# nirajbabar/raytracinginonesemester

Measured on AMD Instinct MI355X. Metric: Mrays/s at 1920x1080x16spp (1/2/4/8 GPU) + PPM max-abs pixel diff, higher is better.
Workload: dtype f32+f64

## Files before the change

raytracinginonesemester_amd/csrc/rt_device.hip:

```cpp

#include <hip/hip_runtime.h>
#include <hip/hip_ext.h>

#include <cfloat>
#include <cmath>
#include <cstdint>
#include <cstdio>
#include <cstdlib>
#include <cstring>
#include <algorithm>
#include <atomic>
#include <functional>
#include <memory>
#include <new>
#include <string>
#include <array>
#include <vector>

#include "rt_common.hpp"
#include "rt_hip_host.hpp"
#include "rt_math.hpp"
#include "rt_ppm.hpp"
#include "rt_scene_pack.hpp"
#include "rt_tilediv.hpp"
// ... 52 lines not shown
    int32_t lane_wide;
    const float* __restrict__ cut;
    int32_t ncut;
    const float* __restrict__ cut2;
    int32_t cut_sub_log2;
    const float4* __restrict__ tri;
    uint32_t* fault;
};

__device__ __forceinline__ f3 scene_bmax(const SceneView& sc) { return mk(sc.bmax[0], sc.bmax[1], sc.bmax[2]); }

struct RenderParams {
    SceneView sc;
    f3 cam_center, cam_p00, cam_du, cam_dv;
    int32_t W, H, spp, max_depth, diffuse_bounce;
    f3 miss;
    const float* __restrict__ jitter;
    int32_t band_rows, band_index, band_count, rows;
    int32_t tile_w, tile_h, tiles_x, tiles_total;
    int32_t lane_samples;
    int32_t half_waves;
    int32_t paired_only;
    int32_t tile_order;
    int32_t spp_log2, tile_w_log2;
    int32_t cull;
    f3 miss_pixel;
    uint32_t* live_count;
    int32_t* live_tiles;
    int32_t* cut_tiles;
    uint32_t* next_count;
    int32_t cut_force;
    int32_t nqueues;
    int32_t queue_cap;
    uint32_t tiles_x_mul;
    float* __restrict__ rgb;
    int32_t* __restrict__ hit_idx;
    float* __restrict__ hit_t;
    uint8_t* __restrict__ p6;
    uint8_t miss_p6[4];
    uint32_t tiles_x_shift;
    uint16_t* __restrict__ tile_cost;
    int32_t* heavy_tiles;
    int32_t heavy_cap;
    uint32_t heavy_ticks[8];
    unsigned long long* ray_count;
    uint32_t* drained;
    uint32_t drain_tag;
    int32_t gate_q8;
};
static_assert(sizeof(RenderParams) == 544, "RenderParams: a field moved");

#include "rt_wave.hpp"
#include "rt_instrument.hpp"
#include "rt_traverse.hpp"
#include "rt_shade.hpp"
#include "rt_prepass.hpp"
#include "rt_query.hpp"
#include "rt_multihit.hpp"
#include "rt_closest.hpp"
#include "rt_path.hpp"
#include "rt_refit.hpp"
#include "rt_rebuild.hpp"

__device__ __forceinline__ int work_length(const RenderParams& P, int q, int& heavy) {
    heavy = 0;
    if (P.heavy_cap > 0)
        for (int k = 0; k < NCLASS; ++k) heavy += min((int)ldc_u32(P.live_count + heavy_counter(k, q)), P.heavy_cap);
    const int slot = P.sc.ncut > 0 ? CUT_SLOT0 + q : q;
    return heavy + (int)ldc_u32(&P.live_count[slot * COUNTER_STRIDE]);
}

__device__ __forceinline__ int work_tile(const RenderParams& P, int q, int e, int heavy, int& cls) {
    const uint32_t* list;
    cls = NCLASS;
    if (e < heavy) {
        int k = 0;
        for (; k < NCLASS - 1; ++k) {
            const int n = min((int)ldc_u32(P.live_count + heavy_counter(k, q)), P.heavy_cap);
            if (e < n) break;
            e -= n;
        }
        list = reinterpret_cast<const uint32_t*>(P.heavy_tiles) + ((size_t)k * 8 + q) * P.heavy_cap;
        cls = k;
    } else {
        e -= heavy;
        list = reinterpret_cast<const uint32_t*>(P.sc.ncut > 0 ? P.cut_tiles : P.live_tiles) + (size_t)q * P.queue_cap;
    }
    return (int)ldc_u32(list + e);
}

__device__ __forceinline__ uint32_t dequeue(uint32_t* head, uint32_t lane) {
    uint32_t v = 0;
    if (lane == 0) v = __hip_atomic_fetch_add(head, 1u, __ATOMIC_RELAXED, __HIP_MEMORY_SCOPE_AGENT);
    return uni(v);
}

template <int MODE, bool D1, int LS = 0>
__device__ __forceinline__ void samples_tile(const RenderParams& P, int tile, uint32_t qw, int t, float* col,
                                             int* kpix, float* park, const int* lds_zero) {
    const uint32_t wv = uni((uint32_t)t) >> 6;
    constexpr int wl = LS != 0 ? 32 : 64;
    const bool on = (t & 63) < wl;
    const int lt = ((int)qw * wl) | (t & (wl - 1));
    bool all_miss = false;
    {
        const int s = lt & (P.spp - 1);
        const int pit = lt >> P.spp_log2;
        int tx, ty;
        if constexpr (D1) {
            ty = (int)tile_div((uint32_t)tile, TileDiv{P.tiles_x_mul, P.tiles_x_shift});
            tx = tile - ty * P.tiles_x;
        } else {
            tx = tile % P.tiles_x;
            ty = tile / P.tiles_x;
        }
#ifndef RT_ROW_PIXELS
        int px, py;
        if (P.tile_w == P.tile_h) {
            px = (pit & 1) | ((pit >> 1) & 2) | ((pit >> 2) & 4) | ((pit >> 3) & 8);
            py = ((pit >> 1) & 1) | ((pit >> 2) & 2) | ((pit >> 3) & 4) | ((pit >> 4) & 8);
        } else {
            px = pit & (P.tile_w - 1);
            py = pit >> P.tile_w_log2;
        }
#else
        const int px = pit & (P.tile_w - 1), py = pit >> P.tile_w_log2;
#endif
        const int x = tx * P.tile_w + px;
        const int r = ty * P.tile_h + py;
        const bool valid = on && x < P.W && r < P.rows;
        const int y = valid ? global_row(P, r) : 0;
        const int pix = valid ? r * P.W + x : -1;
        if (s == 0) kpix[t >> P.spp_log2] = pix;
        const int64_t aov = valid && P.hit_idx ? (int64_t)pix * P.spp + s : -1;
        if constexpr (D1) RT_PHASE_ITEM(park + (wv << 6), (uint32_t)tile * (BLOCK / 64) + qw);
        const f3 c = trace_sample<MODE, D1, LS == 3 ? 2 : 0>(P, valid, x, y, s, aov, park + t,
                                                                             park + (wv << 6));
        if constexpr (D1) RT_PHASE(park + (wv << 6), 1);
        if constexpr (D1) all_miss = P.spp <= 64 && !d1_wave_hit(park + (wv << 6));
        if (!all_miss) {
            const int te = (int)((wv << 6) | __builtin_amdgcn_mbcnt_hi(~0u, __builtin_amdgcn_mbcnt_lo(
                                                      ~0u, (uint32_t)*(const volatile int*)lds_zero)));
            col[3 * te] = c.x;
            col[3 * te + 1] = c.y;
            col[3 * te + 2] = c.z;
        }
    }
    const int t2 = (int)((wv << 6) | __builtin_amdgcn_mbcnt_hi(~0u, __builtin_amdgcn_mbcnt_lo(
                                             ~0u, (uint32_t)*(const volatile int*)lds_zero)));
    if (P.spp <= 64) {
        __builtin_amdgcn_fence(__ATOMIC_RELEASE, "wavefront");
        __builtin_amdgcn_wave_barrier();
        __builtin_amdgcn_fence(__ATOMIC_ACQUIRE, "wavefront");
    } else {
        __syncthreads();
    }
    if (D1 && P.spp <= 64) {
        const int ppw_log2 = 6 - P.spp_log2;
        const float rs = __int_as_float((127 - P.spp_log2) << 23);
        for (int i = t2 & 63; i < (3 << ppw_log2); i += 64) {
            const int ch = i >> ppw_log2, pw = i & ((1 << ppw_log2) - 1);
            const int pix = kpix[(int)(wv << ppw_log2) + pw];
            if (pix < 0) continue;
            const size_t k = (size_t)pix * 3 + ch;
            if (all_miss) {
                const uint32_t m0 = uni((uint32_t)__float_as_int(P.miss_pixel.x)),
                               m1 = uni((uint32_t)__float_as_int(P.miss_pixel.y)),
                               m2 = uni((uint32_t)__float_as_int(P.miss_pixel.z));
                uint32_t b;
                __builtin_memcpy(&b, P.miss_p6, sizeof(b));
                b = uni(b);
                if (P.rgb) P.rgb[k] = __int_as_float((int)(ch == 0 ? m0 : ch == 1 ? m1 : m2));
                if (P.p6) P.p6[k] = (uint8_t)(b >> (8 * ch));
                continue;
            }
            const float* sp = col + 3 * (int)((wv << 6) + ((uint32_t)pw << P.spp_log2)) + ch;
            float acc = 0.f;
            int j = 0;
            for (; j + 16 <= P.spp; j += 16) {
                float s[16];
#pragma unroll
                for (int u = 0; u < 16; ++u) s[u] = sp[3 * (j + u)];
#pragma unroll
                for (int u = 0; u < 16; ++u) acc = acc + s[u];
            }
            for (; j + 4 <= P.spp; j += 4) {
                float s[4];
#pragma unroll
                for (int u = 0; u < 4; ++u) s[u] = sp[3 * (j + u)];
#pragma unroll
                for (int u = 0; u < 4; ++u) acc = acc + s[u];
            }
            for (; j < P.spp; ++j) acc = acc + sp[3 * j];
            const float v = acc * rs;
            if (P.rgb) P.rgb[k] = v;
            if (P.p6) P.p6[k] = rtp::p6_default_sample(v);
        }
        if constexpr (D1) RT_PHASE(park + (wv << 6), 3);
        return;
    }
    if ((t2 & (P.spp - 1)) == 0) {
        const int pix = kpix[t2 >> P.spp_log2];
        if (pix >= 0) {
            f3 acc = mk(0.f, 0.f, 0.f);
            for (int k = 0; k < P.spp; ++k)
                acc = add(acc, mk(col[3 * (t2 + k)], col[3 * (t2 + k) + 1], col[3 * (t2 + k) + 2]));
            const float rs = 1.0f / (float)P.spp;
            const size_t k = (size_t)pix * 3;
            const f3 px = mk(acc.x * rs, acc.y * rs, acc.z * rs);
            if (P.rgb) {
                P.rgb[k] = px.x;
                P.rgb[k + 1] = px.y;
                P.rgb[k + 2] = px.z;
            }
            if (P.p6) {
                P.p6[k] = rtp::p6_default_sample(px.x);
                P.p6[k + 1] = rtp::p6_default_sample(px.y);
                P.p6[k + 2] = rtp::p6_default_sample(px.z);
            }
        }
    }
    if constexpr (D1) RT_PHASE(park + (wv << 6), 3);
}

template <int MODE, bool D1>
__device__ __forceinline__ void pixels_tile(const RenderParams& P, int tile, uint32_t qw, int tid, float* park) {
    const int t = (int)((qw << 6) | (tid & 63));
    const int tx = tile % P.tiles_x, ty = tile / P.tiles_x;
    const int x = tx * P.tile_w + t % P.tile_w;
    const int r = ty * P.tile_h + t / P.tile_w;
    const bool valid = x < P.W && r < P.rows;
    const int y = valid ? global_row(P, r) : 0;
    f3 acc = mk(0.f, 0.f, 0.f);
    if constexpr (D1) RT_PHASE_ITEM(park + (uni((uint32_t)tid) & ~63u), (uint32_t)tile * (BLOCK / 64) + qw);
    for (int s = 0; s < P.spp; ++s) {
        const int64_t aov = valid && P.hit_idx ? ((int64_t)r * P.W + x) * P.spp + s : -1;
        acc = add(acc, trace_sample<MODE, D1>(P, valid, x, y, s, aov, park + tid, park + (uni((uint32_t)tid) & ~63u)));
    }
    if (valid) {
        const float fs = (float)P.spp;
        const size_t k = ((size_t)r * P.W + x) * 3;
        const f3 px = mk(acc.x / fs, acc.y / fs, acc.z / fs);
        if (P.rgb) {
            P.rgb[k] = px.x;
            P.rgb[k + 1] = px.y;
            P.rgb[k + 2] = px.z;
        }
        if (P.p6) {
            P.p6[k] = rtp::p6_default_sample(px.x);
            P.p6[k + 1] = rtp::p6_default_sample(px.y);
            P.p6[k + 2] = rtp::p6_default_sample(px.z);
        }
    }
}

#ifndef RT_RENDER_WAVES
#define RT_RENDER_WAVES 7
#endif
#ifndef RT_BOUNCE_WAVES
#define RT_BOUNCE_WAVES 3
#endif
#ifndef RT_PAIRED_WAVES
#define RT_PAIRED_WAVES 4
#endif
#ifndef RT_RENDER_WAVES_BIG
#define RT_RENDER_WAVES_BIG 8
#endif
struct PairParams {
    RenderParams f[2];
};

__global__ __launch_bounds__(BLOCK) void tile_cull_pair_kernel(PairParams PP) {
    __builtin_amdgcn_s_setprio(3);
    const int nba = (PP.f[0].tiles_total + BLOCK - 1) / BLOCK;
    const bool b = (int)blockIdx.x >= nba;
    const RenderParams& P = b ? PP.f[1] : PP.f[0];
    const int bx = b ? (int)blockIdx.x - nba : (int)blockIdx.x;
    if (bx == 0 && threadIdx.x < COUNTER_SLOTS) P.next_count[threadIdx.x * COUNTER_STRIDE] = 0u;
    cull_tiles(P, bx * BLOCK + (int)threadIdx.x);
}

__global__ __launch_bounds__(BLOCK) void tile_cut_pair_kernel(PairParams PP) {
    __shared__ CutScratch scratch[BLOCK / 64];
    __builtin_amdgcn_s_setprio(3);
    const uint32_t lane = lane_id();
    const int wib = (int)uni(threadIdx.x / 64);
    const int wave = (int)(blockIdx.x * (BLOCK / 64)) + wib;
    const int waves = (int)(gridDim.x * (BLOCK / 64)) / 2;
    const RenderParams& P = (wave & 1) ? PP.f[1] : PP.f[0];
    float box[6] = {0.f, 0.f, 0.f, -1.f, -1.f, -1.f};
    int max_len;
    const bool test = cut_setup(P, lane, box, max_len);
    for (int p = wave >> 1;; p += waves) {
        const int q = p % P.nqueues, g = p / P.nqueues;
        if (CUT_GROUP * g >= max_len) break;
        (void)cut_unit(P, lane, q, g, test, box, scratch[wib]);
    }
}

__device__ __forceinline__ int pair_tile(const RenderParams& A, const RenderParams& B, int q, int e, int& which,
                                         int& cls) {
    for (int k = 0; k < NCLASS; ++k) {
        const int na = A.heavy_cap > 0 ? min((int)ldc_u32(A.live_count + heavy_counter(k, q)), A.heavy_cap) : 0;
        if (e < na) {
            which = 0;
            cls = k;
            return (int)ldc_u32(reinterpret_cast<const uint32_t*>(A.heavy_tiles) + ((size_t)k * 8 + q) * A.heavy_cap + e);
        }
        e -= na;
        const int nb = B.heavy_cap > 0 ? min((int)ldc_u32(B.live_count + heavy_counter(k, q)), B.heavy_cap) : 0;
        if (e < nb) {
            which = 1;
            cls = k;
            return (int)ldc_u32(reinterpret_cast<const uint32_t*>(B.heavy_tiles) + ((size_t)k * 8 + q) * B.heavy_cap + e);
        }
        e -= nb;
    }
    cls = NCLASS;
    const int ra = (int)ldc_u32(&A.live_count[(A.sc.ncut > 0 ? CUT_SLOT0 + q : q) * COUNTER_STRIDE]);
    which = e < ra ? 0 : 1;
    const RenderParams& X = e < ra ? A : B;
    if (e >= ra) e -= ra;
    return (int)ldc_u32(reinterpret_cast<const uint32_t*>(X.sc.ncut > 0 ? X.cut_tiles : X.live_tiles) +
                        (size_t)q * X.queue_cap + e);
}

template <int MODE, bool SAMPLES, bool D1, int WAVES, int LS, bool PAIR>
__device__ __forceinline__ void render_tiles_body() {
    constexpr int WPT = BLOCK / 64;
    __shared__ float col[SAMPLES ? BLOCK * 3 : 1];
    __shared__ int kpix[SAMPLES ? BLOCK : 1];
    __shared__ float park[D1 ? PARK_SLOTS * BLOCK
                             : (MODE == RT_KERNEL_LANE || (MODE & MODE_DEEP) != 0 ? 1 : LANE_LDS_CAP * BLOCK)];
    __shared__ uint32_t t_start[WPT], t_item[WPT];
    __shared__ int lds_zero;
    __shared__ uint32_t block_item;
    if constexpr (SAMPLES) lds_zero = 0;
    const uint32_t wv = uni((uint32_t)threadIdx.x) >> 6;
    for (bool first = true;; first = false) {
        typedef const __attribute__((address_space(4))) RenderParams* KernargP;
        KernargP pp = (KernargP)__builtin_amdgcn_kernarg_segment_ptr();
        uint32_t bx = blockIdx.x;
        asm volatile("" : "+s"(pp), "+s"(bx));
        const RenderParams& R0 = *(const RenderParams*)pp;
        const RenderParams& RG = PAIR ? *(const RenderParams*)(pp + 1) : R0;
        const int g = (int)(bx & 7);
        const int q = R0.nqueues == 1 ? 0 : g;
        uint32_t* head = R0.live_count + (HEAD_SLOT0 + g) * COUNTER_STRIDE;
        const bool blockwise = SAMPLES && R0.spp > 64;
        const uint32_t lane = fresh_lane_id();
        RT_HOOK_FRAME_FIRST(first, lane, RG);
        const int tid = (int)((wv << 6) | lane);
        const uint32_t per_queue = (gridDim.x >> 3) * (blockwise ? 1u : (uint32_t)WPT);
        uint32_t j;
        if (first) {
            j = (bx >> 3) * (blockwise ? 1u : (uint32_t)WPT) + (blockwise ? 0u : wv);
        } else if (blockwise) {
            if (tid == 0) block_item = dequeue(head, lane);
            __syncthreads();
            j = per_queue + uni(block_item);
        } else {
            j = per_queue + dequeue(head, lane);
        }
        int heavy;
        int n = work_length(R0, q, heavy);
        if constexpr (PAIR) {
            int hb;
            n += work_length(RG, q, hb);
        }
        const int e = (R0.nqueues == 1 ? g : 0) + (R0.nqueues == 1 ? 8 : 1) * (int)(blockwise ? j : j / WPT);
        if (RG.drained && lane == 0) {
            const int ge = (int)(((int64_t)n * RG.gate_q8) >> 8);
            if (e >= ge && e < ge + (R0.nqueues == 1 ? 8 : 1))
                __hip_atomic_store(RG.drained, RG.drain_tag, __ATOMIC_RELAXED, __HIP_MEMORY_SCOPE_SYSTEM);
        }
        if (e >= n) {
            RT_HOOK_FRAME_LAST(lane, RG);
            break;
        }
        const uint32_t qw = blockwise ? wv : j % WPT;
        int cls;
        KernargP pr = pp;
        int tile;
        if constexpr (PAIR) {
            int which;
            tile = pair_tile(R0, RG, q, e, which, cls);
            pr = pp + which;
        } else {
            tile = work_tile(R0, q, e, heavy, cls);
        }
        const RenderParams& R = *(const RenderParams*)pr;
        if (cls == 0) __builtin_amdgcn_s_setprio(3);
        else if (cls == 1) __builtin_amdgcn_s_setprio(2);
        else if (cls == 2) __builtin_amdgcn_s_setprio(1);
        else __builtin_amdgcn_s_setprio(0);
        RT_HOOK_ITEM_START(wt0);
        if (R.tile_cost && lane == 0) {
            t_start[wv] = (uint32_t)wall_clock64();
            t_item[wv] = (uint32_t)tile * WPT + qw;
        }
        if constexpr (SAMPLES) samples_tile<MODE, D1, LS>(R, tile, qw, tid, col, kpix, park, &lds_zero);
        else pixels_tile<MODE, D1>(R, tile, qw, tid, park);
        if (R.tile_cost && fresh_lane_id() == 0) {
            asm volatile("" ::: "memory");
            const uint32_t d = (uint32_t)wall_clock64() - t_start[wv];
            R.tile_cost[t_item[wv]] = (uint16_t)(d < 0xffffu ? d : 0xffffu);
        }
        RT_HOOK_ITEM_END(wt0, tile, WPT, qw, bx, first, wv);
    }
}

template <int MODE, bool SAMPLES, bool D1, int WAVES = RT_RENDER_WAVES, int LS = 0>
__global__ __launch_bounds__(BLOCK, WAVES) void render_tiles_kernel(RenderParams P) {
    render_tiles_body<MODE, SAMPLES, D1, WAVES, LS, false>();
}

template <int MODE, bool SAMPLES, bool D1, int WAVES = RT_RENDER_WAVES, int LS = 0>
__global__ __launch_bounds__(BLOCK, WAVES) void render_pair_kernel(PairParams P) {
    render_tiles_body<MODE, SAMPLES, D1, WAVES, LS, true>();
}

__global__ __launch_bounds__(BLOCK) void powf_kernel(const float* __restrict__ x, const float* __restrict__ y, int n,
                                                     float* __restrict__ out) {
    const int i = (int)(blockIdx.x * BLOCK + threadIdx.x);
    if (i < n) out[i] = ref_powf(x[i], y[i]);
}

__global__ __launch_bounds__(BLOCK) void box_test_kernel(const float* __restrict__ rays, const float* __restrict__ boxes,
                                                         const float* __restrict__ tminmax,
                                                         const float* __restrict__ bmax,
                                                         const uint8_t* __restrict__ active, int n,
                                                         int32_t* __restrict__ out) {
    const int i = (int)(blockIdx.x * BLOCK + threadIdx.x);
    const bool in = i < n;
    const size_t j = (size_t)(in ? i : n - 1);
    const float* R = rays + 6 * j;
    const float* B = boxes + 6 * j;
    f3 bm;
    if (bmax != nullptr) {
        bm = mk(bmax[3 * j], bmax[3 * j + 1], bmax[3 * j + 2]);
    } else {
        bm = mk(fmaxf(fabsf(B[0]), fabsf(B[3])), fmaxf(fabsf(B[1]), fabsf(B[4])), fmaxf(fabsf(B[2]), fabsf(B[5])));
        if (!(B[0] <= B[3] && B[1] <= B[4] && B[2] <= B[5])) bm = mk(INFINITY, INFINITY, INFINITY);
    }
    const BoxP b = {(v2f){B[0], B[3]}, (v2f){B[1], B[4]}, (v2f){B[2], B[5]}};
    const float tmin = tminmax[2 * j], tmax = tminmax[2 * j + 1];
    const RayPre r = make_ray(mk(R[0], R[1], R[2]), mk(R[3], R[4], R[5]), bm, tmin);
    const RayPre rw = make_ray(r.o, r.d, bm);
    const uint64_t act = ballot(in && (active == nullptr || active[j] != 0));
    const int cls = box_classify(r, b, tmax);
    const bool h = box_hit(r, b, tmin, tmax);
    const uint64_t m0 = box_hit_mask<false, false>(rw, b, tmax, act);
    const uint64_t m1 = box_hit_mask<true, false>(rw, b, tmax, act);
    const uint64_t m2 = box_hit_mask<true, true>(rw, b, tmax, act);
    if (in) {
        int32_t* O = out + 5 * j;
        O[0] = h ? 1 : 0;
        O[1] = cls;
        O[2] = lane_in(m0) ? 1 : 0;
        O[3] = lane_in(m1) ? 1 : 0;
        O[4] = lane_in(m2) ? 1 : 0;
// ... 1578 lines not shown
    const int slot = int((s->launches - 1) % rt_scene::kRing);
    HIP_TRY(hipEventSynchronize(s->ev1[slot]));
    uint32_t c[COUNTER_SET_U32];
    const size_t counter_bytes = COUNTER_SET_U32 * sizeof(uint32_t);
    HIP_TRY(hipMemcpy(c, static_cast<const char*>(s->work.p) + ((s->launches - 1) % rt_scene::kSets) * counter_bytes, sizeof(c),
                      hipMemcpyDeviceToHost));
    for (int k = 0; k < 8; ++k) *live += c[k * COUNTER_STRIDE];
    if (heavy) {
        *heavy = 0;
        if (s->last_heavy_cap > 0)
            for (int k = 0; k < 8 * NCLASS; ++k)
                *heavy += std::min<int64_t>(c[(HEAVY_SLOT0 + k) * COUNTER_STRIDE], s->last_heavy_cap);
    }
    return RT_OK;
}
}

extern "C" int rt_live_tiles(const rt_scene* s, int64_t* live, int64_t* total) {
    return live_tiles(s, live, nullptr, total);
}

extern "C" const char* rt_scene_kernel_name(const rt_scene* s) {
    return (s && s->last_kernel) ? s->last_kernel : "";
}

extern "C" int rt_heavy_tiles(const rt_scene* s, int64_t* heavy) {
    if (!heavy) return set_error(RT_ERR_ARG, "rt_heavy_tiles: null argument");
    int64_t live = 0, total = 0;
    *heavy = 0;
    return live_tiles(s, &live, heavy, &total);
}

#ifdef RT_STATS
extern "C" int rt_debug_stats(unsigned long long* out, int reset) {
    HIP_TRY(hipDeviceSynchronize());
    HIP_TRY(hipMemcpyFromSymbol(out, HIP_SYMBOL(g_rt_stats), sizeof(g_rt_stats)));
    if (reset) {
        unsigned long long z[24] = {};
        HIP_TRY(hipMemcpyToSymbol(HIP_SYMBOL(g_rt_stats), z, sizeof(z)));
    }
    return RT_OK;
}
#endif

#ifdef RT_WAVE_TIMES
extern "C" int rt_debug_wave_meta_set(void* dev_ptr) {
    HIP_TRY(hipMemcpyToSymbol(HIP_SYMBOL(g_wave_meta), &dev_ptr, sizeof(dev_ptr)));
    return RT_OK;
}
extern "C" int rt_debug_wave_phase_set(void* dev_ptr) {
    HIP_TRY(hipMemcpyToSymbol(HIP_SYMBOL(g_wave_phase), &dev_ptr, sizeof(dev_ptr)));
    return RT_OK;
}
#ifdef RT_LANE_ITERS
extern "C" int rt_debug_lane_iters_set(void* iters_ptr, void* acc_ptr) {
    HIP_TRY(hipMemcpyToSymbol(HIP_SYMBOL(g_lane_iters), &iters_ptr, sizeof(iters_ptr)));
    HIP_TRY(hipMemcpyToSymbol(HIP_SYMBOL(g_lane_acc), &acc_ptr, sizeof(acc_ptr)));
    return RT_OK;
}
#endif
extern "C" int rt_debug_wave_times_set(void* dev_ptr, void* cut_counts_ptr) {
    HIP_TRY(hipMemcpyToSymbol(HIP_SYMBOL(g_wave_times), &dev_ptr, sizeof(dev_ptr)));
    HIP_TRY(hipMemcpyToSymbol(HIP_SYMBOL(g_cut_counts), &cut_counts_ptr, sizeof(cut_counts_ptr)));
    return RT_OK;
}
#endif
#ifdef RT_FRAME_SPAN
extern "C" int rt_debug_frame_span_set(void* dev_ptr) {
    HIP_TRY(hipMemcpyToSymbol(HIP_SYMBOL(g_frame_span), &dev_ptr, sizeof(dev_ptr)));
    return RT_OK;
}
#endif

extern "C" int rt_kernel_times(const rt_scene* s, float* ms_out, int max, int* n_out) {
    return event_times(s, 0, ms_out, max, n_out);
}

extern "C" int rt_frame_times(const rt_scene* s, float* ms_out, int max, int* n_out) {
    return event_times(s, 2, ms_out, max, n_out);
}

extern "C" int rt_prepass_times(const rt_scene* s, float* ms_out, int max, int* n_out) {
    return event_times(s, 1, ms_out, max, n_out);
}

extern "C" int rt_render(rt_scene* s, const rt_camera* cam, const rt_render_opts* o, float* rgb_host,
                         int32_t* hit_idx_host, float* hit_t_host) {
    if (!s || !cam || !o || !rgb_host) return set_error(RT_ERR_ARG, "rt_render: null argument");
    if ((hit_idx_host == nullptr) != (hit_t_host == nullptr)) return set_error(RT_ERR_ARG, "hit_idx and hit_t go together");
    const int rows = rt_shard_rows(cam->pixel_height, o->band_rows, o->band_index, o->band_count);
    if (rows < 0) return set_error(RT_ERR_ARG, "bad band sharding parameters");
    if (o->spp < 1) return set_error(RT_ERR_ARG, "spp must be >= 1");
    DeviceGuard g(s->device);
    const size_t npx = size_t(rows) * size_t(std::max(cam->pixel_width, 0));
    DevBuf rgb, hi, ht;
    int rc;
    if ((rc = rgb.alloc(npx * 3 * sizeof(float))) != RT_OK) return rc;
    if (hit_idx_host) {
        if ((rc = hi.alloc(npx * size_t(o->spp) * sizeof(int32_t))) != RT_OK) return rc;
        if ((rc = ht.alloc(npx * size_t(o->spp) * sizeof(float))) != RT_OK) return rc;
    }
    HIP_TRY(hipDeviceSynchronize());
    HIP_TRY(hipMemset(s->fault.p, 0, sizeof(uint32_t)));
    HIP_TRY(hipDeviceSynchronize());
    rc = rt_render_device(s, cam, o, static_cast<float*>(rgb.p), static_cast<int32_t*>(hi.p),
                          static_cast<float*>(ht.p), nullptr);
// ... 274 lines not shown
```

raytracinginonesemester_amd/csrc/rt_instrument.hpp:

```cpp
#pragma once

#ifdef RT_STATS
__device__ unsigned long long g_rt_stats[24];
#define RT_STAT(i, n) do { if (lane_id() == 0) atomicAdd(&g_rt_stats[(i)], (unsigned long long)(n)); } while (0)
#else
#define RT_STAT(i, n) do { } while (0)
#endif

#ifdef RT_FRAME_SPAN
__device__ unsigned long long* g_frame_span;
#endif
#ifdef RT_WAVE_TIMES
__device__ unsigned long long* g_wave_times;
__device__ uint32_t* g_wave_meta;
__device__ unsigned long long* g_wave_phase;
__device__ int* g_cut_counts;
#define RT_PHASE_ITEM(park_wave, item)                                                                 \
    do {                                                                                               \
        if (lane_id() == 0) (park_wave)[14 * BLOCK] = __int_as_float((int)(item));                     \
    } while (0)
#define RT_PHASE(park_wave, k)                                                                         \
    do {                                                                                               \
        if (g_wave_phase && lane_id() == 0)                                                            \
            g_wave_phase[(size_t)(uint32_t)__float_as_int((park_wave)[14 * BLOCK]) * 4 + (k)] = wall_clock64(); \
    } while (0)
#else
#define RT_PHASE_ITEM(park_wave, item) do { } while (0)
#define RT_PHASE(park_wave, k) do { } while (0)
#endif

#ifdef RT_LANE_ITERS
__device__ uint32_t* g_lane_iters;
__device__ uint32_t* g_lane_acc;
#endif

#ifdef RT_LANE_ITERS
__device__ __forceinline__ uint32_t wave_max_u32(uint32_t v) {
    for (int off = 32; off > 0; off >>= 1) v = max(v, (uint32_t)__shfl_xor((int)v, off));
    return v;
}
__device__ __forceinline__ uint32_t wave_sum_u32(uint32_t v) {
    for (int off = 32; off > 0; off >>= 1) v += (uint32_t)__shfl_xor((int)v, off);
    return v;
}
__device__ __forceinline__ void lane_iters_note(uint32_t it) {
    if (g_lane_acc == nullptr) return;
    uint32_t* a = g_lane_acc + 4 * ((size_t)blockIdx.x * 256 + threadIdx.x);
    a[1] += it;
    const uint32_t m = wave_max_u32(it);
    if ((threadIdx.x & 63) == 0) {
        a[0] += m;
        a[3] += 1;
    }
}
#define RT_LI_ZERO(hs) ((hs).iters = 0)
#define RT_LI_STEP(hs) (++(hs).iters)
#else
#define RT_LI_ZERO(hs) do { } while (0)
#define RT_LI_STEP(hs) do { } while (0)
#endif

#ifdef RT_FRAME_SPAN
#define RT_HOOK_FRAME_FIRST(first, lane, RG)                                                              \
    do {                                                                                                   \
        if ((first) && (lane) == 0 && g_frame_span)                                                        \
            atomicMin(&g_frame_span[4 * ((RG).drain_tag & 255u)], wall_clock64());                         \
    } while (0)
#define RT_HOOK_FRAME_LAST(lane, RG)                                                                       \
    do {                                                                                                   \
        if ((lane) == 0 && g_frame_span) atomicMax(&g_frame_span[4 * ((RG).drain_tag & 255u) + 1], wall_clock64()); \
    } while (0)
#else
#define RT_HOOK_FRAME_FIRST(first, lane, RG) do { } while (0)
#define RT_HOOK_FRAME_LAST(lane, RG) do { } while (0)
#endif

#ifdef RT_LANE_ITERS
__device__ __forceinline__ void lane_iters_reset() {
    if (g_lane_acc) {
        uint32_t* a = g_lane_acc + 4 * ((size_t)blockIdx.x * 256 + threadIdx.x);
        a[0] = a[1] = a[2] = a[3] = 0;
    }
}
#endif
#ifdef RT_WAVE_TIMES
#ifdef RT_LANE_ITERS
#define RT_HOOK_ITEM_START(wt0)                                                                            \
    const unsigned long long wt0 = wall_clock64();                                                         \
    lane_iters_reset()
#else
#define RT_HOOK_ITEM_START(wt0) const unsigned long long wt0 = wall_clock64()
#endif
__device__ __forceinline__ void item_times_note(unsigned long long wt0, int tile, int wpt, uint32_t qw, uint32_t bx,
                                                bool first, uint32_t wv) {
#ifdef RT_LANE_ITERS
    if (g_lane_iters) {
        const uint32_t* a = g_lane_acc + 4 * ((size_t)blockIdx.x * 256 + threadIdx.x);
        const uint32_t mx = wave_max_u32(a[1]), sm = wave_sum_u32(a[1]);
        if ((threadIdx.x & 63) == 0) {
            g_lane_iters[((size_t)tile * wpt + qw) * 4 + 1] = mx;
            g_lane_iters[((size_t)tile * wpt + qw) * 4 + 2] = sm;
        }
    }
#endif
    if (g_wave_times && fresh_lane_id() == 0) {
        const size_t k = ((size_t)tile * wpt + qw) * 2;
        g_wave_times[k] = wt0;
        g_wave_times[k + 1] = wall_clock64();
#ifdef RT_LANE_ITERS
        if (g_lane_iters) {
            const uint32_t* a = g_lane_acc + 4 * ((size_t)blockIdx.x * 256 + threadIdx.x);
            g_lane_iters[((size_t)tile * wpt + qw) * 4 + 0] = a[0];
            g_lane_iters[((size_t)tile * wpt + qw) * 4 + 3] = a[3];
        }
#endif
        if (g_wave_meta) {
            const uint32_t xcc = __builtin_amdgcn_s_getreg((3 << 11) | 20) & 15u;
            g_wave_meta[(size_t)tile * wpt + qw] = bx << 8 | xcc << 4 | (first ? 4u : 0u) | wv;
        }
    }
}
#define RT_HOOK_ITEM_END(wt0, tile, wpt, qw, bx, first, wv) item_times_note(wt0, tile, wpt, qw, bx, first, wv)
#else
#ifdef RT_LANE_ITERS
#define RT_HOOK_ITEM_START(wt0) lane_iters_reset()
#else
#define RT_HOOK_ITEM_START(wt0) do { } while (0)
#endif
#define RT_HOOK_ITEM_END(wt0, tile, wpt, qw, bx, first, wv) do { } while (0)
#endif
```

raytracinginonesemester_amd/csrc/rt_prepass.hpp:

```cpp
#pragma once

struct TileDirsF {
    float c[3], Dl[3], Dh[3], iDl[3], iDh[3], scale;
    bool usable;
};
__host__ __device__ __forceinline__ TileDirsF tile_dirs_f(const RenderParams& P, int x0, int x1, int y0, int y1) {
    TileDirsF T;
    const float p0[3] = {P.cam_p00.x, P.cam_p00.y, P.cam_p00.z};
    const float du[3] = {P.cam_du.x, P.cam_du.y, P.cam_du.z};
    const float dv[3] = {P.cam_dv.x, P.cam_dv.y, P.cam_dv.z};
    T.c[0] = P.cam_center.x;
    T.c[1] = P.cam_center.y;
    T.c[2] = P.cam_center.z;
    const float pxl = (float)x0 - 1.0f, pxh = (float)x1 + 1.0f, pyl = (float)y0 - 1.0f, pyh = (float)y1 + 1.0f;
    const float pxm = fmaxf(fabsf(pxl), fabsf(pxh)), pym = fmaxf(fabsf(pyl), fabsf(pyh));
    T.scale = 0.0f;
#pragma unroll
    for (int a = 0; a < 3; ++a) {
        const float base = p0[a] - T.c[a];
        const float u0 = pxl * du[a], u1 = pxh * du[a], v0 = pyl * dv[a], v1 = pyh * dv[a];
        const float ulp = 16.0f * 1.1920928955078125e-7f * (fabsf(T.c[a]) + fabsf(p0[a]) + pxm * fabsf(du[a]) + pym * fabsf(dv[a]));
        T.Dl[a] = base + fminf(u0, u1) + fminf(v0, v1) - ulp;
        T.Dh[a] = base + fmaxf(u0, u1) + fmaxf(v0, v1) + ulp;
        T.scale = fmaxf(T.scale, fmaxf(fabsf(T.Dl[a]), fabsf(T.Dh[a])));
// ... 4 lines not shown
        T.Dh[a] += 1.1e-5f * T.scale;
        T.iDl[a] = rcp_approx(T.Dl[a]);
        T.iDh[a] = rcp_approx(T.Dh[a]);
    }
    T.usable = T.scale > 0.0f && T.scale < 1e30f;
    return T;
}

__host__ __device__ __forceinline__ bool tile_misses_box_f(const TileDirsF& T, const float* bx) {
    const float mn[3] = {bx[0], bx[1], bx[2]}, mx[3] = {bx[3], bx[4], bx[5]};
    bool inside = true;
    float mag = 0.0f, imax = 0.0f;
#pragma unroll
    for (int a = 0; a < 3; ++a) {
        const float tol = 1e-4f * (fabsf(mn[a]) + fabsf(mx[a]) + fabsf(T.c[a])) + 1e-30f;
        inside = inside && T.c[a] >= mn[a] - tol && T.c[a] <= mx[a] + tol;
        mag = fmaxf(mag, fabsf(mn[a]) + fabsf(mx[a]) + fabsf(T.c[a]));
    }
    if (inside || !T.usable || !(mn[0] <= mx[0] && mn[1] <= mx[1] && mn[2] <= mx[2]) || !(mag < 1e30f)) return false;
    float entry_min = -INFINITY, exit_max = INFINITY;
#pragma unroll
    for (int a = 0; a < 3; ++a) {
        if (!(T.Dl[a] > 1e-6f * T.scale || T.Dh[a] < -1e-6f * T.scale)) continue;
        imax = fmaxf(imax, fmaxf(fabsf(T.iDl[a]), fabsf(T.iDh[a])));
        const float nA = mn[a] - T.c[a], xA = mx[a] - T.c[a];
        const float ne = T.Dl[a] > 0.0f ? nA : xA, nx = T.Dl[a] > 0.0f ? xA : nA;
        const float e0 = ne * T.iDl[a], e1 = ne * T.iDh[a];
        const float f0 = nx * T.iDl[a], f1 = nx * T.iDh[a];
        entry_min = fmaxf(entry_min, fminf(e0, e1));
        exit_max = fminf(exit_max, fmaxf(f0, f1));
    }
    if (!(exit_max == exit_max) || !(entry_min == entry_min)) return false;
    const float abs_slack = 1e-4f * mag * imax + 1e-30f;
    if (!(abs_slack < 1e30f)) return false;
    if (exit_max < -1e-4f * fabsf(exit_max) - abs_slack) return true;
    return entry_min - exit_max > 1e-4f * (fabsf(entry_min) + fabsf(exit_max)) + abs_slack;
}

__device__ __forceinline__ bool tile_misses_root(const RenderParams& P, int x0, int x1, int y0, int y1) {
    return tile_misses_box_f(tile_dirs_f(P, x0, x1, y0, y1), P.sc.root_box);
}

__device__ __forceinline__ f3 miss_sample_color(const RenderParams& P) {
    if (P.max_depth <= 0) return mk(0.f, 0.f, 0.f);
    return clamp01(add(mk(0.f, 0.f, 0.f), mul(mk(1.f, 1.f, 1.f), P.miss)));
}

__device__ __forceinline__ int global_row(const RenderParams& P, int r) {
    if (P.band_count <= 1) return r;
    const int k = r / P.band_rows, within = r - k * P.band_rows;
    return (P.band_index + k * P.band_count) * P.band_rows + within;
}

constexpr int COUNTER_STRIDE = 64;
#ifndef RT_NCLASS
#define RT_NCLASS 5
#endif
constexpr int NCLASS = RT_NCLASS;
constexpr int NCLASS_D1 = 3;
constexpr int HEAVY_SLOT0 = 9;
constexpr int CUT_SLOT0 = HEAVY_SLOT0 + 8 * NCLASS;
constexpr int HEAD_SLOT0 = CUT_SLOT0 + 8;
constexpr int COUNTER_SLOTS = HEAD_SLOT0 + 8;
constexpr int COUNTER_SET_U32 = COUNTER_SLOTS * COUNTER_STRIDE;
__host__ __device__ constexpr int heavy_counter(int k, int q) { return (HEAVY_SLOT0 + 8 * k + q) * COUNTER_STRIDE; }
__device__ __forceinline__ int queue_of_tile(const RenderParams& P, int tile) {
    if (P.nqueues == 1) return 0;
    if (P.tile_order == RT_TILES_XCD_CHUNK) return (int)((int64_t)tile * 8 / P.tiles_total);
    return (tile / P.tiles_x) & 7;
}

__device__ __forceinline__ void write_culled_tile(const RenderParams& P, int tile, int first, int lanes) {
    const int tx = tile % P.tiles_x, ty = tile / P.tiles_x;
    const int xa = tx * P.tile_w, ra = ty * P.tile_h;
    const int tw = min(xa + P.tile_w, P.W) - xa, th = min(ra + P.tile_h, P.rows) - ra;
    const float mp[3] = {P.miss_pixel.x, P.miss_pixel.y, P.miss_pixel.z};
    if (lanes == 1 && tw == 4 && (xa & 3) == 0 && (P.W & 3) == 0 && ((uintptr_t)P.rgb & 15) == 0 &&
        ((uintptr_t)P.p6 & 3) == 0) {
        const float4 f0 = make_float4(mp[0], mp[1], mp[2], mp[0]), f1 = make_float4(mp[1], mp[2], mp[0], mp[1]),
                     f2 = make_float4(mp[2], mp[0], mp[1], mp[2]);
        const uint32_t b0 = P.miss_p6[0], b1 = P.miss_p6[1], b2 = P.miss_p6[2];
        const uint32_t w0 = b0 | b1 << 8 | b2 << 16 | b0 << 24, w1 = b1 | b2 << 8 | b0 << 16 | b1 << 24,
                       w2 = b2 | b0 << 8 | b1 << 16 | b2 << 24;
        for (int r = ra; r < ra + th; ++r) {
            if (P.rgb) {
                float4* o = reinterpret_cast<float4*>(P.rgb + ((size_t)r * P.W + xa) * 3);
                o[0] = f0;
                o[1] = f1;
                o[2] = f2;
            }
            if (P.p6) {
                uint32_t* q = reinterpret_cast<uint32_t*>(P.p6 + ((size_t)r * P.W + xa) * 3);
                q[0] = w0;
                q[1] = w1;
                q[2] = w2;
            }
        }
    } else {
        for (int i = first; i < tw * th * 3; i += lanes) {
            const int px = i / 3, c = i - 3 * px;
            const int r = ra + px / tw, x = xa + px % tw;
            if (P.rgb) P.rgb[((size_t)r * P.W + x) * 3 + c] = c == 0 ? mp[0] : c == 1 ? mp[1] : mp[2];
            if (P.p6) P.p6[((size_t)r * P.W + x) * 3 + c] = c == 0 ? P.miss_p6[0] : c == 1 ? P.miss_p6[1] : P.miss_p6[2];
        }
    }
    if (P.hit_idx) {
        for (int i = first; i < tw * th * P.spp; i += lanes) {
            const int px = i / P.spp, smp = i - P.spp * px;
            const int r = ra + px / tw, x = xa + px % tw;
            const size_t k = ((size_t)r * P.W + x) * (size_t)P.spp + smp;
            P.hit_idx[k] = -1;
            P.hit_t[k] = -1.0f;
        }
    }
}

__device__ __forceinline__ void append_live(const RenderParams& P, bool live, int tile) {
    const int q = live ? queue_of_tile(P, tile) : 0;
// ... 258 lines not shown
```

Measured before the change: 251,900.

## Prefetch next work item during tracing and cache segment table in LDS

The atomic dequeue of the next tile is now issued right after tracing the current sample, before accumulation and writeback, so its latency overlaps with the remaining work. Each wave builds a per-queue prefix table of segment ends once at the start and keeps it in LDS, which replaces recomputing work_length and walking the heavy-class counters from global memory on every item. Tile lookup becomes a table search. The trade-off is extra LDS use and extra wave barriers, plus new debug fetch-timing hooks.

Result: no change. 253,600, median of 5 (+0.7%).

```diff
diff --git a/raytracinginonesemester_amd/csrc/rt_device.hip b/raytracinginonesemester_amd/csrc/rt_device.hip
--- a/raytracinginonesemester_amd/csrc/rt_device.hip
+++ b/raytracinginonesemester_amd/csrc/rt_device.hip
@@ -128,6 +128,21 @@
 
 #include "rt_wave.hpp"
 #include "rt_instrument.hpp"
+#include "rt_itemtable.hpp"
+
+typedef const __attribute__((address_space(4))) RenderParams* KernargP;
+
+__device__ __forceinline__ uint32_t dequeue_issue(bool blockwise, uint32_t wv) {
+    KernargP pp = (KernargP)__builtin_amdgcn_kernarg_segment_ptr();
+    uint32_t bx = blockIdx.x;
+    asm volatile("" : "+s"(pp), "+s"(bx));
+    uint32_t* head = ((const RenderParams*)pp)->live_count + (HEAD_SLOT0 + (int)(bx & 7)) * COUNTER_STRIDE;
+    uint32_t v = 0;
+    if (fresh_lane_id() == 0 && (!blockwise || wv == 0))
+        v = __builtin_amdgcn_atomic_inc32(head, ~0u, __ATOMIC_RELAXED, "agent");
+    return v;
+}
+
 #include "rt_traverse.hpp"
 #include "rt_shade.hpp"
 #include "rt_prepass.hpp"
@@ -138,47 +153,26 @@
 #include "rt_refit.hpp"
 #include "rt_rebuild.hpp"
 
-__device__ __forceinline__ int work_length(const RenderParams& P, int q, int& heavy) {
-    heavy = 0;
-    if (P.heavy_cap > 0)
-        for (int k = 0; k < NCLASS; ++k) heavy += min((int)ldc_u32(P.live_count + heavy_counter(k, q)), P.heavy_cap);
-    const int slot = P.sc.ncut > 0 ? CUT_SLOT0 + q : q;
-    return heavy + (int)ldc_u32(&P.live_count[slot * COUNTER_STRIDE]);
-}
-
-__device__ __forceinline__ int work_tile(const RenderParams& P, int q, int e, int heavy, int& cls) {
-    const uint32_t* list;
-    cls = NCLASS;
-    if (e < heavy) {
-        int k = 0;
-        for (; k < NCLASS - 1; ++k) {
-            const int n = min((int)ldc_u32(P.live_count + heavy_counter(k, q)), P.heavy_cap);
-            if (e < n) break;
-            e -= n;
-        }
-        list = reinterpret_cast<const uint32_t*>(P.heavy_tiles) + ((size_t)k * 8 + q) * P.heavy_cap;
-        cls = k;
-    } else {
-        e -= heavy;
-        list = reinterpret_cast<const uint32_t*>(P.sc.ncut > 0 ? P.cut_tiles : P.live_tiles) + (size_t)q * P.queue_cap;
-    }
-    return (int)ldc_u32(list + e);
-}
-
-__device__ __forceinline__ uint32_t dequeue(uint32_t* head, uint32_t lane) {
-    uint32_t v = 0;
-    if (lane == 0) v = __hip_atomic_fetch_add(head, 1u, __ATOMIC_RELAXED, __HIP_MEMORY_SCOPE_AGENT);
-    return uni(v);
-}
+__device__ __forceinline__ ItemLists item_lists(const RenderParams& P) {
+    return ItemLists{P.live_count, P.heavy_cap, P.sc.ncut > 0 ? 1 : 0, P.queue_cap};
+}
+
+__device__ __forceinline__ int item_tile(const RenderParams& P, int cls, int q, uint32_t local) {
+    const int32_t* lists = cls < NCLASS ? P.heavy_tiles : P.sc.ncut > 0 ? P.cut_tiles : P.live_tiles;
+    return (int)ldc_u32(reinterpret_cast<const uint32_t*>(lists) + item_seg_base(item_lists(P), cls, q) + local);
+}
+
+typedef const volatile __attribute__((address_space(3))) int* LdsZeroP;
 
 template <int MODE, bool D1, int LS = 0>
-__device__ __forceinline__ void samples_tile(const RenderParams& P, int tile, uint32_t qw, int t, float* col,
-                                             int* kpix, float* park, const int* lds_zero) {
+__device__ __forceinline__ uint32_t samples_tile(const RenderParams& P, int tile, uint32_t qw, int t, float* col,
+                                             int* kpix, float* park, LdsZeroP lds_zero) {
     const uint32_t wv = uni((uint32_t)t) >> 6;
     constexpr int wl = LS != 0 ? 32 : 64;
     const bool on = (t & 63) < wl;
     const int lt = ((int)qw * wl) | (t & (wl - 1));
     bool all_miss = false;
+    uint32_t next;
     {
         const int s = lt & (P.spp - 1);
         const int pit = lt >> P.spp_log2;
@@ -213,17 +207,18 @@
         const f3 c = trace_sample<MODE, D1, LS == 3 ? 2 : 0>(P, valid, x, y, s, aov, park + t,
                                                                              park + (wv << 6));
         if constexpr (D1) RT_PHASE(park + (wv << 6), 1);
+        next = dequeue_issue(P.spp > 64, wv);
         if constexpr (D1) all_miss = P.spp <= 64 && !d1_wave_hit(park + (wv << 6));
         if (!all_miss) {
             const int te = (int)((wv << 6) | __builtin_amdgcn_mbcnt_hi(~0u, __builtin_amdgcn_mbcnt_lo(
-                                                      ~0u, (uint32_t)*(const volatile int*)lds_zero)));
+                                                      ~0u, (uint32_t)*lds_zero)));
             col[3 * te] = c.x;
             col[3 * te + 1] = c.y;
             col[3 * te + 2] = c.z;
         }
     }
     const int t2 = (int)((wv << 6) | __builtin_amdgcn_mbcnt_hi(~0u, __builtin_amdgcn_mbcnt_lo(
-                                             ~0u, (uint32_t)*(const volatile int*)lds_zero)));
+                                             ~0u, (uint32_t)*lds_zero)));
     if (P.spp <= 64) {
         __builtin_amdgcn_fence(__ATOMIC_RELEASE, "wavefront");
         __builtin_amdgcn_wave_barrier();
@@ -273,7 +268,7 @@
             if (P.p6) P.p6[k] = rtp::p6_default_sample(v);
         }
         if constexpr (D1) RT_PHASE(park + (wv << 6), 3);
-        return;
+        return next;
     }
     if ((t2 & (P.spp - 1)) == 0) {
         const int pix = kpix[t2 >> P.spp_log2];
@@ -297,6 +292,7 @@
         }
     }
     if constexpr (D1) RT_PHASE(park + (wv << 6), 3);
+    return next;
 }
 
 template <int MODE, bool D1>
@@ -374,33 +370,6 @@
     }
 }
 
-__device__ __forceinline__ int pair_tile(const RenderParams& A, const RenderParams& B, int q, int e, int& which,
-                                         int& cls) {
-    for (int k = 0; k < NCLASS; ++k) {
-        const int na = A.heavy_cap > 0 ? min((int)ldc_u32(A.live_count + heavy_counter(k, q)), A.heavy_cap) : 0;
-        if (e < na) {
-            which = 0;
-            cls = k;
-            return (int)ldc_u32(reinterpret_cast<const uint32_t*>(A.heavy_tiles) + ((size_t)k * 8 + q) * A.heavy_cap + e);
-        }
-        e -= na;
-        const int nb = B.heavy_cap > 0 ? min((int)ldc_u32(B.live_count + heavy_counter(k, q)), B.heavy_cap) : 0;
-        if (e < nb) {
-            which = 1;
-            cls = k;
-            return (int)ldc_u32(reinterpret_cast<const uint32_t*>(B.heavy_tiles) + ((size_t)k * 8 + q) * B.heavy_cap + e);
-        }
-        e -= nb;
-    }
-    cls = NCLASS;
-    const int ra = (int)ldc_u32(&A.live_count[(A.sc.ncut > 0 ? CUT_SLOT0 + q : q) * COUNTER_STRIDE]);
-    which = e < ra ? 0 : 1;
-    const RenderParams& X = e < ra ? A : B;
-    if (e >= ra) e -= ra;
-    return (int)ldc_u32(reinterpret_cast<const uint32_t*>(X.sc.ncut > 0 ? X.cut_tiles : X.live_tiles) +
-                        (size_t)q * X.queue_cap + e);
-}
-
 template <int MODE, bool SAMPLES, bool D1, int WAVES, int LS, bool PAIR>
 __device__ __forceinline__ void render_tiles_body() {
     constexpr int WPT = BLOCK / 64;
@@ -409,80 +378,95 @@
     __shared__ float park[D1 ? PARK_SLOTS * BLOCK
                              : (MODE == RT_KERNEL_LANE || (MODE & MODE_DEEP) != 0 ? 1 : LANE_LDS_CAP * BLOCK)];
     __shared__ uint32_t t_start[WPT], t_item[WPT];
+    __shared__ uint32_t t_next[WPT];
+    typedef ItemSegs<PAIR ? 2 : 1> Segs;
+    __shared__ uint32_t t_tab[WPT][Segs::N + 1];
     __shared__ int lds_zero;
-    __shared__ uint32_t block_item;
+    RT_HOOK_FETCH_DECL(WPT);
     if constexpr (SAMPLES) lds_zero = 0;
     const uint32_t wv = uni((uint32_t)threadIdx.x) >> 6;
     for (bool first = true;; first = false) {
-        typedef const __attribute__((address_space(4))) RenderParams* KernargP;
         KernargP pp = (KernargP)__builtin_amdgcn_kernarg_segment_ptr();
         uint32_t bx = blockIdx.x;
-        asm volatile("" : "+s"(pp), "+s"(bx));
+        uint32_t wt = wv;
+        asm volatile("" : "+s"(pp), "+s"(bx), "+s"(wt));
         const RenderParams& R0 = *(const RenderParams*)pp;
         const RenderParams& RG = PAIR ? *(const RenderParams*)(pp + 1) : R0;
         const int g = (int)(bx & 7);
         const int q = R0.nqueues == 1 ? 0 : g;
-        uint32_t* head = R0.live_count + (HEAD_SLOT0 + g) * COUNTER_STRIDE;
         const bool blockwise = SAMPLES && R0.spp > 64;
         const uint32_t lane = fresh_lane_id();
         RT_HOOK_FRAME_FIRST(first, lane, RG);
+        RT_HOOK_FETCH_BEGIN(wf0, first, wv);
         const int tid = (int)((wv << 6) | lane);
         const uint32_t per_queue = (gridDim.x >> 3) * (blockwise ? 1u : (uint32_t)WPT);
         uint32_t j;
         if (first) {
             j = (bx >> 3) * (blockwise ? 1u : (uint32_t)WPT) + (blockwise ? 0u : wv);
+            const ItemLists L[2] = {item_lists(R0), item_lists(RG)};
+            uint32_t ends[Segs::N + 1];
+            const uint32_t n = item_table_build<PAIR ? 2 : 1>(
+                L, q, [](const uint32_t* p) { return ldc_u32(p); }, [&](int s, uint32_t end) { ends[s] = end; });
+            ends[Segs::N] = item_gate(n, RG.gate_q8);
+            if (lane == 0) {
+#pragma unroll
+                for (int s = 0; s <= Segs::N; ++s) t_tab[wt][s] = ends[s];
+            }
         } else if (blockwise) {
-            if (tid == 0) block_item = dequeue(head, lane);
             __syncthreads();
-            j = per_queue + uni(block_item);
+            asm volatile("" ::: "memory");
+            j = per_queue + uni(t_next[0]);
         } else {
-            j = per_queue + dequeue(head, lane);
-        }
-        int heavy;
-        int n = work_length(R0, q, heavy);
-        if constexpr (PAIR) {
-            int hb;
-            n += work_length(RG, q, hb);
-        }
-        const int e = (R0.nqueues == 1 ? g : 0) + (R0.nqueues == 1 ? 8 : 1) * (int)(blockwise ? j : j / WPT);
+            asm volatile("" ::: "memory");
+            j = per_queue + uni(t_next[wt]);
+        }
+        RT_HOOK_FETCH_VALUE(wf1, j);
+        __builtin_amdgcn_fence(__ATOMIC_RELEASE, "wavefront");
+        __builtin_amdgcn_wave_barrier();
+        __builtin_amdgcn_fence(__ATOMIC_ACQUIRE, "wavefront");
+        asm volatile("" ::: "memory");
+        const uint32_t e =
+            (R0.nqueues == 1 ? (uint32_t)g : 0u) + (R0.nqueues == 1 ? 8u : 1u) * (blockwise ? j : j / WPT);
         if (RG.drained && lane == 0) {
-            const int ge = (int)(((int64_t)n * RG.gate_q8) >> 8);
-            if (e >= ge && e < ge + (R0.nqueues == 1 ? 8 : 1))
+            const uint32_t ge = t_tab[wt][Segs::N];
+            if (e >= ge && e < ge + (R0.nqueues == 1 ? 8u : 1u))
                 __hip_atomic_store(RG.drained, RG.drain_tag, __ATOMIC_RELAXED, __HIP_MEMORY_SCOPE_SYSTEM);
         }
-        if (e >= n) {
+        uint32_t local;
+        const int seg = item_table_find<PAIR ? 2 : 1>([&](int s) { return uni(t_tab[wt][s]); }, e, local);
+        if (seg == Segs::N) {
             RT_HOOK_FRAME_LAST(lane, RG);
             break;
         }
         const uint32_t qw = blockwise ? wv : j % WPT;
-        int cls;
-        KernargP pr = pp;
-        int tile;
-        if constexpr (PAIR) {
-            int which;
-            tile = pair_tile(R0, RG, q, e, which, cls);
-            pr = pp + which;
-        } else {
-            tile = work_tile(R0, q, e, heavy, cls);
-        }
+        const int cls = Segs::cls(seg);
+        const KernargP pr = pp + Segs::frame(seg);
         const RenderParams& R = *(const RenderParams*)pr;
+        const int tile = item_tile(R, cls, q, local);
         if (cls == 0) __builtin_amdgcn_s_setprio(3);
         else if (cls == 1) __builtin_amdgcn_s_setprio(2);
         else if (cls == 2) __builtin_amdgcn_s_setprio(1);
         else __builtin_amdgcn_s_setprio(0);
         RT_HOOK_ITEM_START(wt0);
+        RT_HOOK_FETCH_NOTE(wf0, wf1, tile, WPT, qw, lane);
         if (R.tile_cost && lane == 0) {
             t_start[wv] = (uint32_t)wall_clock64();
             t_item[wv] = (uint32_t)tile * WPT + qw;
         }
-        if constexpr (SAMPLES) samples_tile<MODE, D1, LS>(R, tile, qw, tid, col, kpix, park, &lds_zero);
-        else pixels_tile<MODE, D1>(R, tile, qw, tid, park);
+        uint32_t next;
+        if constexpr (SAMPLES) {
+            next = samples_tile<MODE, D1, LS>(R, tile, qw, tid, col, kpix, park, (LdsZeroP)&lds_zero);
+        } else {
+            pixels_tile<MODE, D1>(R, tile, qw, tid, park);
+            next = dequeue_issue(false, wv);
+        }
         if (R.tile_cost && fresh_lane_id() == 0) {
             asm volatile("" ::: "memory");
             const uint32_t d = (uint32_t)wall_clock64() - t_start[wv];
             R.tile_cost[t_item[wv]] = (uint16_t)(d < 0xffffu ? d : 0xffffu);
         }
         RT_HOOK_ITEM_END(wt0, tile, WPT, qw, bx, first, wv);
+        if (fresh_lane_id() == 0 && (!blockwise || wv == 0)) t_next[blockwise ? 0 : wv] = next;
     }
 }
 
@@ -2167,6 +2151,10 @@
     HIP_TRY(hipMemcpyToSymbol(HIP_SYMBOL(g_wave_phase), &dev_ptr, sizeof(dev_ptr)));
     return RT_OK;
 }
+extern "C" int rt_debug_wave_fetch_set(void* dev_ptr) {
+    HIP_TRY(hipMemcpyToSymbol(HIP_SYMBOL(g_wave_fetch), &dev_ptr, sizeof(dev_ptr)));
+    return RT_OK;
+}
 #ifdef RT_LANE_ITERS
 extern "C" int rt_debug_lane_iters_set(void* iters_ptr, void* acc_ptr) {
     HIP_TRY(hipMemcpyToSymbol(HIP_SYMBOL(g_lane_iters), &iters_ptr, sizeof(iters_ptr)));
diff --git a/raytracinginonesemester_amd/csrc/rt_instrument.hpp b/raytracinginonesemester_amd/csrc/rt_instrument.hpp
--- a/raytracinginonesemester_amd/csrc/rt_instrument.hpp
+++ b/raytracinginonesemester_amd/csrc/rt_instrument.hpp
@@ -14,6 +14,7 @@
 __device__ unsigned long long* g_wave_times;
 __device__ uint32_t* g_wave_meta;
 __device__ unsigned long long* g_wave_phase;
+__device__ unsigned long long* g_wave_fetch;
 __device__ int* g_cut_counts;
 #define RT_PHASE_ITEM(park_wave, item)                                                                 \
     do {                                                                                               \
@@ -91,8 +92,21 @@
 #else
 #define RT_HOOK_ITEM_START(wt0) const unsigned long long wt0 = wall_clock64()
 #endif
+#define RT_HOOK_FETCH_DECL(wpt) __shared__ unsigned long long t_prev[wpt]
+#define RT_HOOK_FETCH_BEGIN(wf0, first, wv)                                                                \
+    const unsigned long long wf0 = (first) ? wall_clock64() : *(const volatile unsigned long long*)&t_prev[wv]
+#define RT_HOOK_FETCH_VALUE(wf1, j)                                                                        \
+    asm volatile("" : "+s"(j));                                                                            \
+    const unsigned long long wf1 = wall_clock64()
+#define RT_HOOK_FETCH_NOTE(wf0, wf1, tile, wpt, qw, lane)                                                  \
+    do {                                                                                                   \
+        if (g_wave_fetch && (lane) == 0) {                                                                 \
+            g_wave_fetch[((size_t)(tile) * (wpt) + (qw)) * 2] = wf0;                                       \
+            g_wave_fetch[((size_t)(tile) * (wpt) + (qw)) * 2 + 1] = wf1;                                   \
+        }                                                                                                  \
+    } while (0)
 __device__ __forceinline__ void item_times_note(unsigned long long wt0, int tile, int wpt, uint32_t qw, uint32_t bx,
-                                                bool first, uint32_t wv) {
+                                                bool first, uint32_t wv, unsigned long long* t_prev) {
 #ifdef RT_LANE_ITERS
     if (g_lane_iters) {
         const uint32_t* a = g_lane_acc + 4 * ((size_t)blockIdx.x * 256 + threadIdx.x);
@@ -106,7 +120,9 @@
     if (g_wave_times && fresh_lane_id() == 0) {
         const size_t k = ((size_t)tile * wpt + qw) * 2;
         g_wave_times[k] = wt0;
-        g_wave_times[k + 1] = wall_clock64();
+        const unsigned long long wt1 = wall_clock64();
+        g_wave_times[k + 1] = wt1;
+        t_prev[wv] = wt1;
 #ifdef RT_LANE_ITERS
         if (g_lane_iters) {
             const uint32_t* a = g_lane_acc + 4 * ((size_t)blockIdx.x * 256 + threadIdx.x);
@@ -120,7 +136,7 @@
         }
     }
 }
-#define RT_HOOK_ITEM_END(wt0, tile, wpt, qw, bx, first, wv) item_times_note(wt0, tile, wpt, qw, bx, first, wv)
+#define RT_HOOK_ITEM_END(wt0, tile, wpt, qw, bx, first, wv) item_times_note(wt0, tile, wpt, qw, bx, first, wv, t_prev)
 #else
 #ifdef RT_LANE_ITERS
 #define RT_HOOK_ITEM_START(wt0) lane_iters_reset()
@@ -128,4 +144,8 @@
 #define RT_HOOK_ITEM_START(wt0) do { } while (0)
 #endif
 #define RT_HOOK_ITEM_END(wt0, tile, wpt, qw, bx, first, wv) do { } while (0)
+#define RT_HOOK_FETCH_DECL(wpt) do { } while (0)
+#define RT_HOOK_FETCH_BEGIN(wf0, first, wv) do { } while (0)
+#define RT_HOOK_FETCH_VALUE(wf1, j) do { } while (0)
+#define RT_HOOK_FETCH_NOTE(wf0, wf1, tile, wpt, qw, lane) do { } while (0)
 #endif
diff --git a/raytracinginonesemester_amd/csrc/rt_itemtable.hpp b/raytracinginonesemester_amd/csrc/rt_itemtable.hpp
--- /dev/null
+++ b/raytracinginonesemester_amd/csrc/rt_itemtable.hpp
@@ -0,0 +1,79 @@
+#pragma once
+
+#include <stdint.h>
+
+#if defined(__HIPCC__) || defined(__CUDACC__)
+#define RTI_HD __host__ __device__ inline
+#else
+#define RTI_HD inline
+#endif
+
+constexpr int COUNTER_STRIDE = 64;
+#ifndef RT_NCLASS
+#define RT_NCLASS 5
+#endif
+constexpr int NCLASS = RT_NCLASS;
+constexpr int NCLASS_D1 = 3;
+constexpr int HEAVY_SLOT0 = 9;
+constexpr int CUT_SLOT0 = HEAVY_SLOT0 + 8 * NCLASS;
+constexpr int HEAD_SLOT0 = CUT_SLOT0 + 8;
+constexpr int COUNTER_SLOTS = HEAD_SLOT0 + 8;
+constexpr int COUNTER_SET_U32 = COUNTER_SLOTS * COUNTER_STRIDE;
+RTI_HD constexpr int heavy_counter(int k, int q) { return (HEAVY_SLOT0 + 8 * k + q) * COUNTER_STRIDE; }
+
+struct ItemLists {
+    const uint32_t* count;
+    int32_t heavy_cap;
+    int32_t use_cut;
+    int32_t queue_cap;
+};
+
+template <int NF>
+struct ItemSegs {
+    static constexpr int N = NF * (NCLASS + 1);
+    static RTI_HD constexpr int cls(int s) { return s / NF; }
+    static RTI_HD constexpr int frame(int s) { return s % NF; }
+};
+
+template <class Load>
+RTI_HD uint32_t item_seg_count(const ItemLists& L, int cls, int q, Load ld) {
+    if (cls < NCLASS) {
+        const uint32_t cap = L.heavy_cap > 0 ? (uint32_t)L.heavy_cap : 0u;
+        const uint32_t c = ld(L.count + heavy_counter(cls, q));
+        return c < cap ? c : cap;
+    }
+    return ld(L.count + (L.use_cut ? CUT_SLOT0 + q : q) * COUNTER_STRIDE);
+}
+
+RTI_HD size_t item_seg_base(const ItemLists& L, int cls, int q) {
+    return cls < NCLASS ? ((size_t)cls * 8 + (size_t)q) * (size_t)L.heavy_cap : (size_t)q * (size_t)L.queue_cap;
+}
+
+template <int NF, class Load, class Store>
+RTI_HD uint32_t item_table_build(const ItemLists* L, int q, Load ld, Store st) {
+    uint32_t end = 0;
+#pragma unroll
+    for (int s = 0; s < ItemSegs<NF>::N; ++s) {
+        end += item_seg_count(L[ItemSegs<NF>::frame(s)], ItemSegs<NF>::cls(s), q, ld);
+        st(s, end);
+    }
+    return end;
+}
+
+template <int NF, class Load>
+RTI_HD int item_table_find(Load ld, uint32_t e, uint32_t& local) {
+    int seg = 0;
+    uint32_t start = 0;
+#pragma unroll
+    for (int s = 0; s < ItemSegs<NF>::N; ++s) {
+        const uint32_t end = ld(s);
+        if (e >= end) {
+            seg = s + 1;
+            start = end;
+        }
+    }
+    local = e - start;
+    return seg;
+}
+
+RTI_HD uint32_t item_gate(uint32_t n, int32_t gate_q8) { return (uint32_t)(((int64_t)n * gate_q8) >> 8); }
diff --git a/raytracinginonesemester_amd/csrc/rt_prepass.hpp b/raytracinginonesemester_amd/csrc/rt_prepass.hpp
--- a/raytracinginonesemester_amd/csrc/rt_prepass.hpp
+++ b/raytracinginonesemester_amd/csrc/rt_prepass.hpp
@@ -80,18 +80,7 @@
     return (P.band_index + k * P.band_count) * P.band_rows + within;
 }
 
-constexpr int COUNTER_STRIDE = 64;
-#ifndef RT_NCLASS
-#define RT_NCLASS 5
-#endif
-constexpr int NCLASS = RT_NCLASS;
-constexpr int NCLASS_D1 = 3;
-constexpr int HEAVY_SLOT0 = 9;
-constexpr int CUT_SLOT0 = HEAVY_SLOT0 + 8 * NCLASS;
-constexpr int HEAD_SLOT0 = CUT_SLOT0 + 8;
-constexpr int COUNTER_SLOTS = HEAD_SLOT0 + 8;
-constexpr int COUNTER_SET_U32 = COUNTER_SLOTS * COUNTER_STRIDE;
-__host__ __device__ constexpr int heavy_counter(int k, int q) { return (HEAVY_SLOT0 + 8 * k + q) * COUNTER_STRIDE; }
+#include "rt_itemtable.hpp"
 __device__ __forceinline__ int queue_of_tile(const RenderParams& P, int tile) {
     if (P.nqueues == 1) return 0;
     if (P.tile_order == RT_TILES_XCD_CHUNK) return (int)((int64_t)tile * 8 / P.tiles_total);
```
